# boomluo02/EEMFlow

Measured on AMD Instinct MI355X. Metric: frames/sec + EPE, EEMFlow 1280×720 dt1, 1/2/4/8 MI355X, higher is better.
Workload: dtype f32; 1 GPU; EEMFlow inference, HREM 1280x720 dt1, batch=1 per GPU (BASELINE configs[1]); synthetic 20%-dense voxel pairs resident in HBM, seeded Kaiming weights; height=720, width=1280, batch_per_gpu=1, hip_graph=True, streams_per_gpu=2, coalesced_frames=10, frames_in_flight_hint=2, preheat_steps=200, input_pairs_rotated=8, input_bytes_rotated=294912000, parallelism=replicas x1: frames sharded over ranks, no data-path collective

## Files before the change

eemflow_amd/_lib.py:

```python
import ctypes
import os

_HERE = os.path.dirname(os.path.abspath(__file__))
LIB_PATH = os.environ.get("EEM_LIB_PATH") or os.path.join(_HERE, "libeemflow_hip.so")

_c_float_p = ctypes.c_void_p


class KernelStat(ctypes.Structure):
    _fields_ = [("name", ctypes.c_char * 48), ("flops", ctypes.c_double), ("bytes", ctypes.c_double),
                ("ms", ctypes.c_float), ("blocks", ctypes.c_int), ("pipe", ctypes.c_int), ("reserved", ctypes.c_int)]


_SIGNATURES = {
    "eemflow_abi_version": (ctypes.c_int, []),
    "eemflow_last_error": (ctypes.c_char_p, []),
    "eemflow_create": (ctypes.c_int, [ctypes.c_int, ctypes.POINTER(ctypes.c_void_p)]),
    "eemflow_destroy": (None, [ctypes.c_void_p]),
    "eemflow_load_weights": (ctypes.c_int, [ctypes.c_void_p, _c_float_p, ctypes.c_size_t, ctypes.c_int, ctypes.c_int]),
    "eemflow_update_weights": (ctypes.c_int, [ctypes.c_void_p, _c_float_p, ctypes.c_size_t, ctypes.c_void_p]),
    "eemflow_forward_train": (ctypes.c_int, [ctypes.c_void_p, _c_float_p, _c_float_p, ctypes.c_int, ctypes.c_int, ctypes.c_int,
                                             _c_float_p, ctypes.c_int, ctypes.c_int, ctypes.POINTER(ctypes.c_int64), ctypes.c_void_p]),
    "eemflow_backward": (ctypes.c_int, [ctypes.c_void_p, ctypes.c_int64, _c_float_p, _c_float_p, _c_float_p, _c_float_p,
                                        ctypes.c_void_p]),
    "eemflow_backward_forms": (ctypes.c_int, [ctypes.c_void_p, ctypes.c_char_p, ctypes.c_size_t]),
    "eemflow_sequence_loss": (ctypes.c_int, [_c_float_p, _c_float_p, _c_float_p, ctypes.c_int, ctypes.c_int, ctypes.c_int, ctypes.c_float,
                                             _c_float_p, ctypes.c_void_p, ctypes.c_void_p]),
    "eemflow_set_image_size": (ctypes.c_int, [ctypes.c_void_p, ctypes.c_int, ctypes.c_int, ctypes.POINTER(ctypes.c_int * 4)]),
    "eemflow_use_graph": (ctypes.c_int, [ctypes.c_void_p, ctypes.c_int]),
    "eemflow_set_frames_in_flight": (ctypes.c_int, [ctypes.c_void_p, ctypes.c_int]),
    "eemflow_set_deferred_input_norm": (ctypes.c_int, [ctypes.c_void_p, ctypes.c_int]),
    "eemflow_graph_stats": (ctypes.c_int, [ctypes.c_void_p, ctypes.POINTER(ctypes.c_longlong * 3)]),
    "eemflow_forward": (ctypes.c_int, [ctypes.c_void_p, _c_float_p, _c_float_p, ctypes.c_int, ctypes.c_int, ctypes.c_int,
                                       _c_float_p, ctypes.c_int, ctypes.c_int, ctypes.c_void_p]),
    "eemflow_forward_many": (ctypes.c_int, [ctypes.c_void_p, ctypes.c_int, ctypes.POINTER(ctypes.c_void_p), ctypes.POINTER(ctypes.c_void_p),
                                            ctypes.POINTER(ctypes.c_void_p), ctypes.c_int, ctypes.c_int, ctypes.c_int, ctypes.c_int,
                                            ctypes.c_void_p]),
    "eemflow_forward_stream": (ctypes.c_int, [ctypes.c_void_p, ctypes.c_int, ctypes.POINTER(ctypes.c_void_p), ctypes.POINTER(ctypes.c_void_p),
                                              ctypes.c_int, ctypes.c_int, ctypes.c_int, ctypes.c_int, ctypes.c_int, ctypes.c_void_p]),
    "eemflow_forward_stream_bidir": (ctypes.c_int, [ctypes.c_void_p, ctypes.c_int, ctypes.POINTER(ctypes.c_void_p), ctypes.POINTER(ctypes.c_void_p),
                                                    ctypes.POINTER(ctypes.c_void_p), ctypes.c_int, ctypes.c_int, ctypes.c_int, ctypes.c_int,
                                                    ctypes.c_int, ctypes.c_void_p]),
    "eemflow_stream_reset": (ctypes.c_int, [ctypes.c_void_p]),
    "eemflow_stream_pending": (ctypes.c_int, [ctypes.c_void_p, ctypes.POINTER(ctypes.c_int)]),
    "eemflow_time_kernels": (ctypes.c_int, [ctypes.c_void_p, _c_float_p, _c_float_p, ctypes.c_int, ctypes.c_int, ctypes.c_int,
                                            _c_float_p, ctypes.c_int, ctypes.c_int, ctypes.c_int, ctypes.POINTER(KernelStat),
                                            ctypes.c_int, ctypes.POINTER(ctypes.c_int), ctypes.c_void_p]),
    "eemflow_get_stage": (ctypes.c_int, [ctypes.c_void_p, ctypes.c_char_p, _c_float_p, ctypes.c_size_t,
                                         ctypes.POINTER(ctypes.c_int * 4), ctypes.c_void_p]),
    "eemflow_decoder": (ctypes.c_int, [ctypes.c_void_p, ctypes.c_int, _c_float_p, ctypes.c_int, ctypes.c_int, ctypes.c_int,
                                       _c_float_p, ctypes.c_void_p]),
    "eemflow_local_corr53": (ctypes.c_int, [_c_float_p, _c_float_p, ctypes.c_int, ctypes.c_int, ctypes.c_int, ctypes.c_int,
                                            _c_float_p, ctypes.c_void_p]),
    "eemflow_upsample_bilinear": (ctypes.c_int, [_c_float_p, _c_float_p, ctypes.c_int, ctypes.c_int, ctypes.c_int,
                                                 ctypes.c_int, ctypes.c_int, ctypes.c_void_p]),
    "eraft_corr_lookup_bwd": (ctypes.c_int, [_c_float_p, _c_float_p, ctypes.c_int, ctypes.c_int, ctypes.c_int, _c_float_p,
                                             _c_float_p, _c_float_p, _c_float_p, ctypes.c_void_p]),
    "eraft_corr_pyramid_bwd": (ctypes.c_int, [_c_float_p, _c_float_p, _c_float_p, _c_float_p, _c_float_p, _c_float_p, ctypes.c_int,
                                              ctypes.c_int, ctypes.c_int, ctypes.c_int, _c_float_p, _c_float_p, ctypes.c_void_p]),
    "eraft_convex_upsample_bwd": (ctypes.c_int, [_c_float_p, _c_float_p, _c_float_p, ctypes.c_int, ctypes.c_int, ctypes.c_int,
                                                 _c_float_p, _c_float_p, ctypes.c_void_p]),
    "eemplus_warp_bwd": (ctypes.c_int, [_c_float_p, _c_float_p, _c_float_p, ctypes.c_int, ctypes.c_int, ctypes.c_int, ctypes.c_int,
                                        ctypes.c_int, _c_float_p, _c_float_p, ctypes.c_void_p]),
    "eemflow_flow_error": (ctypes.c_int, [_c_float_p, _c_float_p, ctypes.c_void_p, ctypes.c_int, ctypes.c_int, ctypes.c_int,
# ... 144 lines not shown
```

eemflow_amd/csrc/api.hip:

```cpp
#include <stdarg.h>
#include <stdlib.h>
#include <string.h>

#include <string>
#include <vector>

#include "ctx.h"
#include <mutex>

static thread_local char g_err[512] = "";
thread_local int eem_last_grid_blocks = 0, eem_last_grid_threads = 0, eem_last_pipe = 0;

void eem_set_error(const char* fmt, ...) {
    va_list ap;
    va_start(ap, fmt);
    vsnprintf(g_err, sizeof(g_err), fmt, ap);
    va_end(ap);
}

extern "C" const char* eemflow_last_error(void) { return g_err; }
extern "C" int eemflow_abi_version(void) { return 1; }

extern "C" int eemflow_create(int device, eemflow_ctx** out) {
    EEM_REQUIRE(out != nullptr, "eemflow_create: out is NULL");
    int ndev = 0;
    EEM_HIP_CHECK(hipGetDeviceCount(&ndev));
    EEM_REQUIRE(device >= 0 && device < ndev, "eemflow_create: device %d of %d", device, ndev);
    EEM_HIP_CHECK(hipSetDevice(device));
    hipDeviceProp_t prop;
    EEM_HIP_CHECK(hipGetDeviceProperties(&prop, device));
    EEM_REQUIRE(strncmp(prop.gcnArchName, "gfx950", 6) == 0,
                "this library is built for gfx950 (MI355X) only; device %d is %s", device, prop.gcnArchName);
    eemflow_ctx* c = new eemflow_ctx();
    c->device = device;
    hipError_t e = hipMalloc(&c->taps, sizeof(kTaps53));
    if (e == hipSuccess) e = hipMemcpy(c->taps, kTaps53, sizeof(kTaps53), hipMemcpyHostToDevice);
    if (e == hipSuccess) e = hipMalloc(&c->zero_page, 4096);
    if (e == hipSuccess) e = hipMemset(c->zero_page, 0, 4096);
    if (e == hipSuccess) e = hipMalloc(&c->io_table, 3 * EEM_MAX_COALESCE * sizeof(void*));
    if (e == hipSuccess) e = hipMemset(c->io_table, 0, 3 * EEM_MAX_COALESCE * sizeof(void*));
    if (e != hipSuccess) {
        eem_set_error("eemflow_create: %s", hipGetErrorString(e));
        delete c;
        return EEM_ERR_HIP;
    }
    *out = c;
    return EEM_OK;
}

extern "C" void eemflow_destroy(eemflow_ctx* c) {
    if (!c) return;
    (void)hipSetDevice(c->device);
    drop_graph(c);
    DevBuf* bufs[] = {&c->a1, &c->f11, &c->a2, &c->b2, &c->f12, &c->a3, &c->b3, &c->f13, &c->flowcat, &c->coarse, &c->carry,
                      &c->padded, &c->fuse_scratch, &c->g_a1, &c->g_f11, &c->g_a2, &c->g_b2, &c->g_f12, &c->g_a3, &c->g_b3, &c->g_f13,
                      &c->g_flowcat, &c->g_coarse, &c->g_flow, &c->ups_tmp, &c->grad_flat, &c->adam_m, &c->adam_v, &c->scalars};
    for (DevBuf* b : bufs) if (b->p) (void)hipFree(b->p);
    for (int k = 0; k < 3; ++k) {
        if (c->ppart[k].p) (void)hipFree(c->ppart[k].p);
        DevBuf* kb[] = {&c->pool[k], &c->cat[k], &c->ta[k], &c->tb[k], &c->tc[k], &c->td[k], &c->t64[k], &c->t32[k],
                        &c->g_pool[k], &c->g_cat[k], &c->g_ta[k], &c->g_tb[k], &c->g_tc[k], &c->g_td[k], &c->g_t64[k], &c->g_t32[k]};
        for (DevBuf* b : kb) if (b->p) (void)hipFree(b->p);
    }
    if (c->cstream) { (void)hipStreamSynchronize(c->cstream); (void)hipStreamDestroy(c->cstream); }
// ... 725 lines not shown
```

eemflow_amd/csrc/common.h:

```cpp
#pragma once
#include <hip/hip_runtime.h>
#include <cstdio>
#include <cstdlib>
#include <stdint.h>
#include <stdio.h>

#include <type_traits>

#include "../../include/eemflow_hip.h"

typedef float f32x2 __attribute__((ext_vector_type(2)));
typedef float f32x4 __attribute__((ext_vector_type(4)));
typedef float f32x16 __attribute__((ext_vector_type(16)));
typedef double f64x2 __attribute__((ext_vector_type(2)));
typedef unsigned u32x4 __attribute__((ext_vector_type(4)));

#define EEM_OK 0
#define EEM_ERR_ARG 1
#define EEM_ERR_HIP 2
#define EEM_ERR_STATE 3

void eem_set_error(const char* fmt, ...);

extern thread_local const char* eem_conv_form;

#define EEM_HIP_CHECK(expr)                                                            \
    do {                                                                               \
        hipError_t _e = (expr);                                                        \
        if (_e != hipSuccess) {                                                        \
            eem_set_error("%s failed: %s (%s:%d)", #expr, hipGetErrorString(_e),       \
                          __FILE__, __LINE__);                                         \
            return EEM_ERR_HIP;                                                        \
        }                                                                              \
    } while (0)

#define EEM_REQUIRE(cond, ...)                                                         \
    do {                                                                               \
        if (!(cond)) {                                                                 \
            eem_set_error(__VA_ARGS__);                                                \
            return EEM_ERR_ARG;                                                        \
        }                                                                              \
    } while (0)

__host__ __device__ static inline int ceil_div(int a, int b) { return (a + b - 1) / b; }

extern thread_local int eem_last_grid_blocks, eem_last_grid_threads, eem_last_pipe;
#define EEM_NOTE_GRID(blocks, threads) do { eem_last_grid_blocks = (int)(blocks); eem_last_grid_threads = (int)(threads); } while (0)
#define EEM_NOTE_PIPE(p) do { eem_last_pipe = (int)(p); } while (0)

template <int I, int N, class F>
__device__ __forceinline__ void static_for(F&& f) {
    if constexpr (I < N) {
        f(std::integral_constant<int, I>{});
        static_for<I + 1, N>(f);
    }
}
template <int N>
__device__ __forceinline__ void wait_vmcnt() {
    asm volatile("s_waitcnt vmcnt(%0)" ::"n"(N > 63 ? 63 : N) : "memory");
}

__device__ static inline unsigned xcd_logical_block(unsigned bid, unsigned nblocks_padded) {
    const unsigned cpx = nblocks_padded >> 3;
    return (bid & 7u) * cpx + (bid >> 3);
}

template <int CTRL>
__device__ static __forceinline__ float dpp_add(float v) {
    return v + __int_as_float(__builtin_amdgcn_update_dpp(0, __float_as_int(v), CTRL, 0xF, 0xF, true));
}
template <int SW>
__device__ static __forceinline__ float lane_group_sum(float v) {
    static_assert(SW == 4 || SW == 8 || SW == 16, "group width");
    v = dpp_add<0xB1>(v);
    v = dpp_add<0x4E>(v);
    if (SW >= 8) v = dpp_add<0x141>(v);
    if (SW >= 16) v = dpp_add<0x140>(v);
    return v;
}

static inline int enc_blocks_per_xcd(const char* tag, int dflt) {
    char name[48];
    snprintf(name, sizeof name, "EEM_ENC_PER_XCD_%s", tag);
    const char* e = getenv(name);
    if (!e) e = getenv("EEM_ENC_PER_XCD");
    const int v = e ? atoi(e) : 0;
    return v > 0 ? v : dflt;
}
struct TileCoord { int bx, by, n; };
struct TileRange { int first, count; };
__device__ static inline TileRange block_tile_range(int T, unsigned bid, unsigned nblocks) {
    const int cpx = (T + 7) >> 3;
    const int xcd = bid & 7, kb = bid >> 3, gb = nblocks >> 3;
    const int r0 = xcd * cpx, r1 = min(r0 + cpx, T);
    const int per = (cpx + gb - 1) / gb;
    const int f = r0 + kb * per;
    const int cnt = min(per, r1 - f);
    return TileRange{f, cnt > 0 ? cnt : 0};
}
__device__ static inline TileCoord tile_coord(int lt, int tiles_x, int tiles_y) {
    return TileCoord{lt % tiles_x, (lt / tiles_x) % tiles_y, lt / (tiles_x * tiles_y)};
// ... 217 lines not shown
```

eemflow_amd/csrc/conv_bx3.hip:

```cpp
#include "common.h"

namespace {

#define LDS_PTR(p) ((__attribute__((address_space(3))) void*)(p))
#define GLB_PTR(p) ((const __attribute__((address_space(1))) void*)(p))

typedef unsigned u32x4 __attribute__((ext_vector_type(4)));
typedef __bf16 bf16x8 __attribute__((ext_vector_type(8)));

template <int CIN, int COUT>
struct BxCfg {
    static constexpr int TH = 4, NPIX = 32, WAVES = 4;
    static constexpr int MT = COUT / 32;
    static constexpr int NC16 = CIN / 16;
    static constexpr int KSTEPS = 9 * NC16;
    static constexpr int IN_ROWS = 2 * (TH - 1) + 3;
    static constexpr int ROWP = 68;
    static constexpr int PPR = ROWP / 4;
    static constexpr int PLANE = IN_ROWS * ROWP;
    static constexpr int PIECES = CIN * IN_ROWS * PPR;
    static constexpr int NI = (PIECES + WAVES * 64 - 1) / (WAVES * 64);
    static constexpr int LDS_FLOATS = NI * WAVES * 256;
    static constexpr int RING = 3;
};

__device__ __forceinline__ bf16x8 as_bf(const u32x4& v) { return __builtin_bit_cast(bf16x8, v); }

__device__ __forceinline__ void split8(const float (&x)[8], u32x4& p0, u32x4& p1, u32x4& p2) {
#pragma unroll
    for (int d = 0; d < 4; ++d) {
        const float xa = x[2 * d], xb = x[2 * d + 1];
        const float ra = xa - __uint_as_float(__float_as_uint(xa) & 0xffff0000u), rb = xb - __uint_as_float(__float_as_uint(xb) & 0xffff0000u);
        const float sa = ra - __uint_as_float(__float_as_uint(ra) & 0xffff0000u), sb = rb - __uint_as_float(__float_as_uint(rb) & 0xffff0000u);
        p0[d] = __builtin_amdgcn_perm(__float_as_uint(xb), __float_as_uint(xa), 0x07060302u);
        p1[d] = __builtin_amdgcn_perm(__float_as_uint(rb), __float_as_uint(ra), 0x07060302u);
        p2[d] = __builtin_amdgcn_perm(__float_as_uint(sb), __float_as_uint(sa), 0x07060302u);
    }
}

__device__ __forceinline__ void split_pair(const float (&x)[8], int d, u32x4& p0, u32x4& p1, u32x4& p2) {
    const float xa = x[2 * d], xb = x[2 * d + 1];
    const float ra = xa - __uint_as_float(__float_as_uint(xa) & 0xffff0000u), rb = xb - __uint_as_float(__float_as_uint(xb) & 0xffff0000u);
    const float sa = ra - __uint_as_float(__float_as_uint(ra) & 0xffff0000u), sb = rb - __uint_as_float(__float_as_uint(rb) & 0xffff0000u);
    p0[d] = __builtin_amdgcn_perm(__float_as_uint(xb), __float_as_uint(xa), 0x07060302u);
    p1[d] = __builtin_amdgcn_perm(__float_as_uint(rb), __float_as_uint(ra), 0x07060302u);
    p2[d] = __builtin_amdgcn_perm(__float_as_uint(sb), __float_as_uint(sa), 0x07060302u);
}

template <int CIN, int COUT>
__global__ __launch_bounds__(256, (CIN == 16 ? 4 : 2)) void bx3_s2_kernel(EncConvArgs a, const u32x4* __restrict__ wq) {
    using C = BxCfg<CIN, COUT>;
    __shared__ __attribute__((aligned(16))) float lds[C::LDS_FLOATS];
    const int tid = threadIdx.x;
    const int lane = tid & 63;
    const int wave = __builtin_amdgcn_readfirstlane(tid >> 6);
    ENC_ARGS_NOW(a);
    const unsigned lid = xcd_logical_block(blockIdx.x, gridDim.x);
    if (lid >= (unsigned)(a.tiles_x * a.tiles_y * a.nimg)) return;
    const int bx = lid % a.tiles_x, by = (lid / a.tiles_x) % a.tiles_y;
    const int n = lid / (a.tiles_x * a.tiles_y);
    const int row = wave;
    const int j = lane & 31, g = lane >> 5;

    const u32x4* wsrc = wq + lane;
    u32x4 wv[C::RING][3][C::MT];
#pragma unroll
    for (int s = 0; s < C::RING; ++s)
#pragma unroll
        for (int p = 0; p < 3; ++p)
#pragma unroll
            for (int m = 0; m < C::MT; ++m) wv[s][p][m] = wsrc[((s * 3 + p) * C::MT + m) * 64];

    const int oy0 = by * C::TH, ox0 = bx * C::NPIX;
    const int gy0 = oy0 * 2 - 1, gxa = ox0 * 2 - 4;
    const float* src = a.in0 + (size_t)n * CIN * a.hin * a.win;
#pragma unroll
    for (int k = 0; k < C::NI; ++k) {
// ... 23 lines not shown
        for (int e = 0; e < 8; ++e) x[e] = bl[(c16 * 16 + e) * C::PLANE + (t / 3) * C::ROWP + (t % 3)];
    };
    asm volatile("s_waitcnt vmcnt(0)" ::: "memory");
    __builtin_amdgcn_s_barrier();
    float x[2][8];
    u32x4 b[2][3];
    read_x(0, x[0]);
    if (C::KSTEPS > 1) read_x(1, x[1]);
    split8(x[0], b[0][0], b[0][1], b[0][2]);
#pragma unroll
    for (int s = 0; s < C::KSTEPS; ++s) {
        const int cur = s & 1, nxt = cur ^ 1;
        u32x4(&w)[3][C::MT] = wv[s % C::RING];
        if (s + 2 < C::KSTEPS) read_x(s + 2, x[cur]);
        __builtin_amdgcn_sched_barrier(0);
#pragma unroll
        for (int q = 0; q < 6; ++q) {
            constexpr int PW[6] = {2, 1, 0, 1, 0, 0}, PB[6] = {0, 1, 2, 0, 1, 0};
#pragma unroll
            for (int m = 0; m < C::MT; ++m)
                acc[m] = __builtin_amdgcn_mfma_f32_32x32x16_bf16(as_bf(w[PW[q]][m]), as_bf(b[cur][PB[q]]), acc[m], 0, 0, 0);
            if (q < 4 && s + 1 < C::KSTEPS) split_pair(x[nxt], q, b[nxt][0], b[nxt][1], b[nxt][2]);
            __builtin_amdgcn_sched_barrier(0);
        }
        if (s + C::RING < C::KSTEPS) {
#pragma unroll
            for (int p = 0; p < 3; ++p)
#pragma unroll
                for (int m = 0; m < C::MT; ++m) w[p][m] = wsrc[(((s + C::RING) * 3 + p) * C::MT + m) * 64];
        }
        __builtin_amdgcn_sched_barrier(0);
    }

    const int oy = oy0 + row, ox = ox0 + j;
    const int hw = a.hout * a.wout;
    float* dst = a.out + (size_t)n * COUT * hw;
    const bool full = oy0 + C::TH <= a.hout && ox0 + C::NPIX <= a.wout;
#pragma unroll
    for (int m = 0; m < C::MT; ++m) {
        const int co0 = m * 32 + 4 * g;
        const unsigned lane_bo = (unsigned)((co0 * a.hout + oy) * a.wout + ox) * 4u;
#pragma unroll
        for (int r = 0; r < 16; ++r) {
            float v = acc[m][r];
            if (a.act) v = fmaxf(v, 0.1f * v);
            const int dco = (r & 3) + 8 * (r >> 2);
            if (full) {
                char* rb = reinterpret_cast<char*>(dst) + (size_t)dco * hw * 4;
                *reinterpret_cast<float*>(rb + lane_bo) = v;
            } else if (oy < a.hout && ox < a.wout) {
                dst[(size_t)(co0 + dco) * hw + oy * a.wout + ox] = v;
            }
        }
    }
}

__global__ void bx3_wt_kernel(const float* __restrict__ w, int cin, int cout, unsigned* __restrict__ out, int total) {
    const int i = blockIdx.x * blockDim.x + threadIdx.x;
    if (i >= total) return;
    const int nc16 = cin / 16, mt_n = cout / 32;
    const int d = i & 3, lane = (i >> 2) & 63;
    int rest = i >> 8;
    const int mt = rest % mt_n; rest /= mt_n;
    const int s = rest;
    const int t = s / nc16, c16 = s % nc16;
    const int co = mt * 32 + (lane & 31), c = c16 * 16 + 8 * (lane >> 5) + 2 * d;
    unsigned lo[3], hi[3];
    for (int h = 0; h < 2; ++h) {
        const float x = w[((size_t)co * cin + c + h) * 9 + t];
        const float x0 = __uint_as_float(__float_as_uint(x) & 0xffff0000u), r = x - x0;
        const float x1 = __uint_as_float(__float_as_uint(r) & 0xffff0000u), q = r - x1;
        unsigned* dst = h ? hi : lo;
        dst[0] = __float_as_uint(x0) >> 16; dst[1] = __float_as_uint(x1) >> 16; dst[2] = __float_as_uint(q) >> 16;
    }
    for (int p = 0; p < 3; ++p) out[((((size_t)s * 3 + p) * mt_n + mt) * 64 + lane) * 4 + d] = (hi[p] << 16) | lo[p];
}

template <int CIN, int COUT, int KGT>
struct B1Cfg {
    static constexpr int TH = 4, NPIX = 32, KG = KGT, WAVES = 4 * KG, THREADS = 64 * WAVES;
    static constexpr int MT = COUT / 32;
    static constexpr int NC16 = CIN / 16, NCG = NC16 / KG;
    static constexpr int KLOC = 9 * NCG;
    static constexpr int NG = CIN / 8;
    static constexpr int IN_ROWS = TH + 2, COLS = 40, QPR = COLS / 4;
    static constexpr int ITEMS = NG * IN_ROWS * QPR;
    static constexpr int GPLANE = IN_ROWS * COLS;
    static constexpr int TILE_U4 = 3 * NG * GPLANE;
    static constexpr int SLOT_U4 = 3 * MT * 64;
    static constexpr int NQ = 3 * MT;
    static constexpr int RING = KG == 1 ? 6 : 4, AHEAD = RING - 1;
    static constexpr int LDS_U4 = TILE_U4 + KG * RING * SLOT_U4;
    static_assert(ITEMS <= THREADS && NC16 % KG == 0 && NQ <= 8 && (KG == 1 || MT == 2), "one staging item per thread; two groups finish one cout tile each");
    static_assert(KG == 1 || MT * 4 * 64 * 4 <= TILE_U4, "partial-sum exchange fits the dead input tile");
    static_assert(LDS_U4 * 16 <= 160 * 1024, "LDS");
};

template <int N>
__device__ __forceinline__ void bx_wait_vm(int nrow) {
    if (nrow == 2) asm volatile("s_waitcnt vmcnt(%0)" ::"n"(2 * N) : "memory");
    else if (nrow == 1) asm volatile("s_waitcnt vmcnt(%0)" ::"n"(N) : "memory");
    else asm volatile("s_waitcnt vmcnt(0)" ::: "memory");
}

template <int CIN, int COUT, int KGT>
__global__ __launch_bounds__((64 * 4 * KGT), (KGT == 1 ? 2 : 1)) void bx3_s1_kernel(EncConvArgs a, const u32x4* __restrict__ wq) {
// ... 104 lines not shown
        f32x16* xch = reinterpret_cast<f32x16*>(lds);
        xch[((1 - kg) * 4 + row) * 64 + lane] = kg == 0 ? acc[1] : acc[0];
        __syncthreads();
        f32x16 mine = kg == 0 ? acc[0] : acc[1];
        const f32x16 other = xch[(kg * 4 + row) * 64 + lane];
        const int co0 = kg * 32 + 4 * g;
        if (oy < a.hout && ox < a.wout) {
#pragma unroll
            for (int r = 0; r < 16; ++r) {
                const int co = co0 + (r & 3) + 8 * (r >> 2);
                float v = mine[r] + other[r] + a.bias[co];
                if (a.act) v = fmaxf(v, 0.1f * v);
                dst[(size_t)co * hw + oy * a.wout + ox] = v;
            }
        }
    } else {
        if (oy < a.hout && ox < a.wout) {
#pragma unroll
            for (int m = 0; m < C::MT; ++m)
#pragma unroll
                for (int r = 0; r < 16; ++r) {
                    const int co = m * 32 + 4 * g + (r & 3) + 8 * (r >> 2);
                    float v = acc[m][r] + a.bias[co];
                    if (a.act) v = fmaxf(v, 0.1f * v);
                    dst[(size_t)co * hw + oy * a.wout + ox] = v;
                }
        }
    }
}

template <int CIN, int COUT, int KGT>
int bx3_s1_launch_t(const EncConvArgs& a0, hipStream_t stream) {
    using C = B1Cfg<CIN, COUT, KGT>;
    EncConvArgs a = a0;
    a.tiles_x = ceil_div(a.wout, C::NPIX);
    a.tiles_y = ceil_div(a.hout, C::TH);
    dim3 grid((unsigned)ceil_div(a.tiles_x * a.tiles_y * a.nimg, 8) * 8);
    EEM_NOTE_GRID(grid.x, C::THREADS);
    EEM_NOTE_PIPE(1);
    hipLaunchKernelGGL((bx3_s1_kernel<CIN, COUT, KGT>), grid, dim3(C::THREADS), 0, stream, a, reinterpret_cast<const u32x4*>(a.wbx3));
    EEM_HIP_CHECK(hipGetLastError());
    return EEM_OK;
}

template <int CIN, int COUT>
int bx3_launch_t(const EncConvArgs& a0, hipStream_t stream) {
    using C = BxCfg<CIN, COUT>;
    EncConvArgs a = a0;
    a.tiles_x = ceil_div(a.wout, C::NPIX);
    a.tiles_y = ceil_div(a.hout, C::TH);
    dim3 grid((unsigned)ceil_div(a.tiles_x * a.tiles_y * a.nimg, 8) * 8);
    EEM_NOTE_GRID(grid.x, 256);
    EEM_NOTE_PIPE(1);
    hipLaunchKernelGGL((bx3_s2_kernel<CIN, COUT>), grid, dim3(256), 0, stream, a, reinterpret_cast<const u32x4*>(a.wbx3));
    EEM_HIP_CHECK(hipGetLastError());
    return EEM_OK;
}

}

bool bx3_shape(int cin, int cout, int stride) {
    return (stride == 2 && ((cin == 16 && cout == 32) || (cin == 32 && cout == 64))) || (stride == 1 && cin == cout && (cin == 32 || cin == 64));
}

size_t bx3_packed_floats(int cin, int cout) { return (size_t)9 * (cin / 16) * 3 * (cout / 32) * 64 * 4; }

int bx3_transform_launch(const float* w, int cin, int cout, float* packed, hipStream_t stream) {
    const int total = 9 * (cin / 16) * (cout / 32) * 64 * 4;
    hipLaunchKernelGGL(bx3_wt_kernel, dim3(ceil_div(total, 256)), dim3(256), 0, stream, w, cin, cout, reinterpret_cast<unsigned*>(packed), total);
    EEM_HIP_CHECK(hipGetLastError());
    return EEM_OK;
}

bool bx3_supported(int cin, int cout, int stride, const EncConvArgs& a) {
    const char* off = getenv("EEM_NO_BX3");
    if (off && off[0] == '1') return false;
    if (stride == 2 && cin == 32) {
        const char* m = getenv("EEM_NO_BX3_64");
        if (m && m[0] == '1') return false;
    }
    if (stride == 1) {
        const char* m = getenv("EEM_BX3_S1");
        const int mask = m ? atoi(m) : 0;
        if (!(mask & (cin == 32 ? 1 : 2))) return false;
    }
    return bx3_shape(cin, cout, stride) && a.wbx3 && a.gate == nullptr && a.pool_partial == nullptr && a.res == nullptr && (a.win & 3) == 0 &&
           (a.act == 0 || a.act == 1) && (((uintptr_t)a.in0) & 15) == 0 && (size_t)cin * a.hin * a.win * 4 < (1u << 31);
}

int bx3_launch(int cin, int stride, const EncConvArgs& a, hipStream_t stream) {
    if (cin == 64) return bx3_s1_launch_t<64, 64, 2>(a, stream);
    if (cin == 32 && stride == 2) return bx3_launch_t<32, 64>(a, stream);
    if (cin == 32) return bx3_s1_launch_t<32, 32, 1>(a, stream);
    return bx3_launch_t<16, 32>(a, stream);
}
```

eemflow_amd/csrc/ctx.h:

```cpp
#pragma once
#include <stdarg.h>
#include <string.h>

#include <string>
#include <vector>

#include "../../include/eemflow_hip.h"
#include "common.h"
#include "gconv.h"
#include "eraft_kernels.h"
#include "wnc.h"

inline constexpr int kTaps53[53] = {0,  2,  4,  6,  8,  10, 12, 14, 16, 18, 20, 21, 22, 23, 24, 26, 28, 29,
                                    30, 31, 32, 33, 34, 36, 38, 39, 40, 41, 42, 44, 46, 47, 48, 49, 50, 51,
                                    52, 54, 56, 57, 58, 59, 60, 62, 64, 66, 68, 70, 72, 74, 76, 78, 80};
constexpr int kNTaps = 53;
constexpr int kDecIn = kNTaps + 16;
constexpr int kDecW = 100;

struct TailW {
    size_t wpk = 0, bias = 0;
    int cin = 0, cout = 0, ksize = 3;
};

// ... 119 lines not shown
        int stream_nvol = 0;
        int stream_carry = 0, stream_slot = 0;
        int stream_bidir = 0;
        bool operator==(const Key& o) const {
            return batch == o.batch && in_h == o.in_h && in_w == o.in_w && out_h == o.out_h && out_w == o.out_w &&
                   pad[0] == o.pad[0] && pad[1] == o.pad[1] && pad[2] == o.pad[2] && pad[3] == o.pad[3] && aligned16 == o.aligned16 &&
                   io_frames == o.io_frames && deferred_norm == o.deferred_norm && stream_nvol == o.stream_nvol &&
                   stream_carry == o.stream_carry && stream_slot == o.stream_slot && stream_bidir == o.stream_bidir;
        }
    };
    struct GraphEntry {
        Key key;
        Shape shape;
        bool f13_skipped = false;
        bool a1_skipped = false;
        hipGraph_t graph = nullptr;
        hipGraphExec_t exec = nullptr;
        long last_use = 0;
    };
    static constexpr int kMaxGraphs = 4;
    std::vector<GraphEntry> graphs;
    long graph_clock = 0;
    const void** io_table = nullptr;
    const void* io_host[3 * EEM_MAX_COALESCE] = {};
    int io_host_n = 0;
    int cur_io_frames = 0;
    void* io_stream = nullptr;
    long graph_captures = 0, graph_replays = 0, io_updates = 0;
};

struct Hook {
    hipStream_t st = nullptr;
    bool timing = false;
    int reps = 1;
    bool repeat = false;
    int pass = 0;
    size_t slot = 0;
    std::vector<hipEvent_t> evs;
    std::vector<eemflow_kernel_stat> stats;

    static bool skipped(const char* name);

    template <class F>
    int run(const char* name, double flops, double bytes, F&& launch) {
#ifdef EEM_DIAG
        if (skipped(name)) {
            static const float spin = [] { const char* e = getenv("EEM_SKIP_SPIN_US"); return e ? (float)atof(e) : 0.f; }();
            return spin > 0.f ? spin_launch(spin, st) : EEM_OK;
        }
#endif
        if (!timing) return launch(st);
        if (repeat) {
            if (evs.size() < 2) { evs.resize(2, nullptr); EEM_HIP_CHECK(hipEventCreate(&evs[0])); EEM_HIP_CHECK(hipEventCreate(&evs[1])); }
            eem_last_grid_blocks = eem_last_grid_threads = eem_last_pipe = 0;
            int rc = launch(st);
            if (rc != EEM_OK) return rc;
            EEM_HIP_CHECK(hipEventRecord(evs[0], st));
            for (int i = 0; i < reps; ++i)
                if ((rc = launch(st)) != EEM_OK) return rc;
            EEM_HIP_CHECK(hipEventRecord(evs[1], st));
            EEM_HIP_CHECK(hipEventSynchronize(evs[1]));
            float ms = 0.f;
            EEM_HIP_CHECK(hipEventElapsedTime(&ms, evs[0], evs[1]));
            eemflow_kernel_stat ks;
            memset(&ks, 0, sizeof(ks));
            strncpy(ks.name, name, sizeof(ks.name) - 1);
            ks.flops = flops; ks.bytes = bytes; ks.ms = ms;
            ks.blocks = eem_last_grid_blocks;
            ks.pipe = eem_last_pipe;
            stats.push_back(ks);
            return EEM_OK;
        }
        if (evs.size() < 2 * (slot + 1)) {
            evs.resize(2 * (slot + 1), nullptr);
            EEM_HIP_CHECK(hipEventCreate(&evs[2 * slot]));
            EEM_HIP_CHECK(hipEventCreate(&evs[2 * slot + 1]));
        }
        eem_last_grid_blocks = eem_last_grid_threads = eem_last_pipe = 0;
        EEM_HIP_CHECK(hipEventRecord(evs[2 * slot], st));
        const int rc = launch(st);
        if (rc != EEM_OK) return rc;
        EEM_HIP_CHECK(hipEventRecord(evs[2 * slot + 1], st));
        if (pass == 0) {
            eemflow_kernel_stat ks;
            memset(&ks, 0, sizeof(ks));
            strncpy(ks.name, name, sizeof(ks.name) - 1);
            ks.flops = flops; ks.bytes = bytes; ks.ms = 0.f;
            ks.blocks = eem_last_grid_blocks;
            ks.pipe = eem_last_pipe;
            stats.push_back(ks);
        }
        ++slot;
        return EEM_OK;
    }
    int collect(bool count);
    void release();
};

extern thread_local unsigned long g_realloc_events;
int ensure(DevBuf& b, size_t floats);
int refresh_wino(eemflow_ctx* c, hipStream_t);
int ensure_bx3(eemflow_ctx* c, int l, hipStream_t st, const float** w_out);
int ensure_s2r(eemflow_ctx* c, int l, hipStream_t st, const float** w_out);
int ensure_wino(eemflow_ctx* c, int l, int dir, int batch, hipStream_t st, const float** w_out, int* f4_out);
int ensure_dec_wnc(eemflow_ctx* c, hipStream_t st);
int ensure_train_wino(eemflow_ctx* c, int batch, hipStream_t st);
int ensure_forward_wino(eemflow_ctx* c, int batch, hipStream_t st);
void drop_graph(eemflow_ctx* c);
int compute_shape(eemflow_ctx* c, int batch, int in_h, int in_w, int out_h, int out_w, Shape* s, int nimg = -1);
int alloc_workspace(eemflow_ctx* c, const Shape& s);

bool s2r_wanted();
bool bx3_wanted(int l);
bool dec_wnc_wanted(const eemflow_ctx* c, int gw, int batch);
int run_decoders(eemflow_ctx* c, int k0, int k1, const float* const cat[3], int batch, int h, int w, float* flow_dst,
                 int flow_ctotal, int kbase, Hook& hk);
int run_enc_layer(eemflow_ctx* c, const Shape& s, int li, const float* e1, const float* e2, Hook& hk, const void* const* io,
                  const float* prepadded, bool may_skip_store);
int run_forward(eemflow_ctx* c, const Shape& s, const float* e1, const float* e2, float* out, Hook& hk,
                const void* const* io = nullptr, const float* prepadded = nullptr);
```

include/eemflow_hip.h:

```cpp
#ifndef EEMFLOW_HIP_H
#define EEMFLOW_HIP_H

#include <stddef.h>
#include <stdint.h>

#ifdef __cplusplus
extern "C" {
#endif
typedef struct eemflow_ctx eemflow_ctx;
typedef struct eraft_ctx eraft_ctx;
typedef struct eemplus_ctx eemplus_ctx;

#if defined(__GNUC__)
#pragma GCC visibility push(default)
#endif

int eemflow_abi_version(void);

const char* eemflow_last_error(void);

int eemflow_create(int device, eemflow_ctx** out);
void eemflow_destroy(eemflow_ctx* ctx);

int eemflow_load_weights(eemflow_ctx* ctx, const float* flat_host, size_t nfloats, int n_first_channels,
                         int groups);

int eemflow_update_weights(eemflow_ctx* ctx, const float* flat_device, size_t nfloats, void* stream);

int eemflow_set_image_size(eemflow_ctx* ctx, int height, int width, int pad_out[4]);

int eemflow_use_graph(eemflow_ctx* ctx, int enable);

int eemflow_set_frames_in_flight(eemflow_ctx* ctx, int n);

int eemflow_set_deferred_input_norm(eemflow_ctx* ctx, int enable);

int eemflow_graph_stats(eemflow_ctx* ctx, long long out3[3]);

int eemflow_forward(eemflow_ctx* ctx, const float* events1, const float* events2, int batch, int in_h,
                    int in_w, float* flow_out, int out_h, int out_w, void* stream);

int eemflow_forward_many(eemflow_ctx* ctx, int nframes, const float* const* events1, const float* const* events2,
                         float* const* flow_out, int in_h, int in_w, int out_h, int out_w, void* stream);

#define EEM_STREAM_MAX_VOLUMES 16

int eemflow_forward_stream(eemflow_ctx* ctx, int nvol, const float* const* volumes, float* const* flow_out, int nflow, int in_h,
                           int in_w, int out_h, int out_w, void* stream);

#define EEM_STREAM_BIDIR_MAX_VOLUMES 8

int eemflow_forward_stream_bidir(eemflow_ctx* ctx, int nvol, const float* const* volumes, float* const* flow_fw_out,
                                 float* const* flow_bw_out, int nflow, int in_h, int in_w, int out_h, int out_w, void* stream);

int eemflow_stream_reset(eemflow_ctx* ctx);

int eemflow_stream_pending(eemflow_ctx* ctx, int* out);

typedef struct eemflow_kernel_stat {
    char name[48];
    double flops;
    double bytes;
    float ms;
    int blocks;
    int pipe;
    int reserved;
} eemflow_kernel_stat;
int eemflow_time_kernels(eemflow_ctx* ctx, const float* events1, const float* events2, int batch, int in_h,
                         int in_w, float* flow_out, int out_h, int out_w, int reps, eemflow_kernel_stat* stats,
                         int max_stats, int* nstats, void* stream);

int eemflow_get_stage(eemflow_ctx* ctx, const char* name, float* dst, size_t dst_capacity_floats,
                      int dims_out[4], void* stream);

int eemflow_decoder(eemflow_ctx* ctx, int k, const float* x, int batch, int h, int w, float* out, void* stream);

int eemflow_local_corr53(const float* f1, const float* f2, int batch, int c, int h, int w, float* out,
                         void* stream);

int eemflow_upsample_bilinear(const float* in, float* out, int nc, int h, int w, int oh, int ow, void* stream);

int eemflow_flow_error(const float* flow_gt, const float* flow_pred, const float* event_img, int h, int w, int max_row,
                       double* out5, void* stream);

int eemflow_flow_error_many(int n, const float* const* flow_gt, const float* const* flow_pred, const float* const* event_img, int h,
                            int w, int max_row, double* out5n, void* stream);

int eemflow_fb_check_many(int n, const float* const* flow_fw, const float* const* flow_bw, float* const* mask_fw_out,
                          float* const* mask_bw_out, int h, int w, float alpha1, float alpha2, int mode, void* stream);

int eemflow_flow_to_image_many(int n, const float* const* flow, uint8_t* const* image_out, double* stats, int h, int w, int bgr,
                               void* stream);

int eemflow_event_image_many(int n, const float* const* volume, const float* const* norm, int bins, int h, int w,
                             uint8_t* const* image_out, double* stats, int bgr, void* stream);

int eemflow_voxelize(const double* events, int64_t n, int bins, int h, int w, int normalize, float* grid,
                     int64_t* idx_left, int64_t* idx_right, void* stream);

int eemflow_voxelize_pair(const double* events1, int64_t n1, const double* events2, int64_t n2, int bins, int h, int w,
                          int normalize, float* grid1, float* grid2, void* stream);

int eemflow_voxelize_many(int nsets, const double* const* events, const int64_t* n_events, int bins, int h, int w, int normalize,
                          float* const* grids, void* stream);


int eemflow_forward_train(eemflow_ctx* ctx, const float* events1, const float* events2, int batch, int in_h, int in_w,
                          float* flow_out, int out_h, int out_w, int64_t* serial_out, void* stream);
int eemflow_backward(eemflow_ctx* ctx, int64_t serial, const float* events1, const float* events2, const float* dflow,
                     float* grad_out, void* stream);

int eemflow_backward_forms(eemflow_ctx* ctx, char* dst, size_t capacity);

int eemflow_sequence_loss(const float* flow, const float* flow_gt, const float* valid, int batch, int h, int w, float weight,
                          float* dflow_out, double* stats6, void* stream);

int eemflow_forward_backward(eemflow_ctx* ctx, const float* events1, const float* events2, const float* flow_gt,
                             const float* valid, int batch, int in_h, int in_w, int out_h, int out_w,
                             float loss_weight, float* flow_out, float* grad_out, double* stats_out, void* stream);
// ... 154 lines not shown
```

Measured before the change: 11050 frames/s.

## Add lean stride-2 bx3 conv kernel with padded LDS planes and packed split

```diff
diff --git a/eemflow_amd/_lib.py b/eemflow_amd/_lib.py
--- a/eemflow_amd/_lib.py
+++ b/eemflow_amd/_lib.py
@@ -9,7 +9,7 @@
 
 class KernelStat(ctypes.Structure):
     _fields_ = [("name", ctypes.c_char * 48), ("flops", ctypes.c_double), ("bytes", ctypes.c_double),
-                ("ms", ctypes.c_float), ("blocks", ctypes.c_int), ("pipe", ctypes.c_int), ("reserved", ctypes.c_int)]
+                ("ms", ctypes.c_float), ("blocks", ctypes.c_int), ("pipe", ctypes.c_int), ("form", ctypes.c_int)]
 
 
 _SIGNATURES = {
diff --git a/eemflow_amd/csrc/api.hip b/eemflow_amd/csrc/api.hip
--- a/eemflow_amd/csrc/api.hip
+++ b/eemflow_amd/csrc/api.hip
@@ -9,7 +9,7 @@
 #include <mutex>
 
 static thread_local char g_err[512] = "";
-thread_local int eem_last_grid_blocks = 0, eem_last_grid_threads = 0, eem_last_pipe = 0;
+thread_local int eem_last_grid_blocks = 0, eem_last_grid_threads = 0, eem_last_pipe = 0, eem_last_form = 0;
 
 void eem_set_error(const char* fmt, ...) {
     va_list ap;
diff --git a/eemflow_amd/csrc/common.h b/eemflow_amd/csrc/common.h
--- a/eemflow_amd/csrc/common.h
+++ b/eemflow_amd/csrc/common.h
@@ -44,9 +44,10 @@
 
 __host__ __device__ static inline int ceil_div(int a, int b) { return (a + b - 1) / b; }
 
-extern thread_local int eem_last_grid_blocks, eem_last_grid_threads, eem_last_pipe;
+extern thread_local int eem_last_grid_blocks, eem_last_grid_threads, eem_last_pipe, eem_last_form;
 #define EEM_NOTE_GRID(blocks, threads) do { eem_last_grid_blocks = (int)(blocks); eem_last_grid_threads = (int)(threads); } while (0)
 #define EEM_NOTE_PIPE(p) do { eem_last_pipe = (int)(p); } while (0)
+#define EEM_NOTE_FORM(f) do { eem_last_form = (int)(f); } while (0)
 
 template <int I, int N, class F>
 __device__ __forceinline__ void static_for(F&& f) {
diff --git a/eemflow_amd/csrc/conv_bx3.hip b/eemflow_amd/csrc/conv_bx3.hip
--- a/eemflow_amd/csrc/conv_bx3.hip
+++ b/eemflow_amd/csrc/conv_bx3.hip
@@ -22,7 +22,31 @@
     static constexpr int NI = (PIECES + WAVES * 64 - 1) / (WAVES * 64);
     static constexpr int LDS_FLOATS = NI * WAVES * 256;
     static constexpr int RING = 3;
+    static constexpr int PLANE_L = 640;
+    static constexpr int PPL = PLANE_L / 4;
+    static constexpr int PERIOD = 5;
+    static_assert(CIN * PPL == NI * WAVES * 64 && CIN * PLANE_L == LDS_FLOATS, "the padded planes fill today's LDS exactly");
+    static_assert(PERIOD * WAVES * 64 == 8 * PPL && NI % PERIOD == 0, "five rounds are eight planes");
+    static_assert((CIN - 9) * (PLANE_L / 64) <= 255, "read2st64 offsets (channel c16 * 16 + e; 8 g is the lane's) are 8 bits of 64-dword strides");
 };
+
+struct BxPiece { unsigned c, ry, q; };
+__host__ __device__ constexpr BxPiece bx_piece(unsigned p) {
+    const unsigned c = (((p >> 5) & 0xffu) * 205u) >> 10;
+    unsigned rem = p - c * 160u;
+    rem = rem < 152u ? rem : 152u;
+    const unsigned ry = (rem * 241u) >> 12;
+    return BxPiece{c, ry, rem - ry * 17u};
+}
+constexpr bool bx_piece_check() {
+    for (unsigned p = 0; p < 32 * 160; ++p) {
+        const BxPiece x = bx_piece(p);
+        const unsigned rem = p % 160 < 152 ? p % 160 : 152;
+        if (x.c != p / 160 || x.ry != rem / 17 || x.q != rem % 17) return false;
+    }
+    return true;
+}
+static_assert(bx_piece_check(), "bx_piece");
 
 __device__ __forceinline__ bf16x8 as_bf(const u32x4& v) { return __builtin_bit_cast(bf16x8, v); }
 
@@ -152,6 +176,155 @@
                 dst[(size_t)(co0 + dco) * hw + oy * a.wout + ox] = v;
             }
         }
+    }
+}
+
+__device__ __forceinline__ void split_pk(const f32x2 x, int d, u32x4& p0, u32x4& p1, u32x4& p2) {
+    typedef unsigned u32x2 __attribute__((ext_vector_type(2)));
+    const f32x2 r = x - __builtin_bit_cast(f32x2, __builtin_bit_cast(u32x2, x) & 0xffff0000u);
+    const f32x2 q = r - __builtin_bit_cast(f32x2, __builtin_bit_cast(u32x2, r) & 0xffff0000u);
+    p0[d] = __builtin_amdgcn_perm(__float_as_uint(x[1]), __float_as_uint(x[0]), 0x07060302u);
+    p1[d] = __builtin_amdgcn_perm(__float_as_uint(r[1]), __float_as_uint(r[0]), 0x07060302u);
+    p2[d] = __builtin_amdgcn_perm(__float_as_uint(q[1]), __float_as_uint(q[0]), 0x07060302u);
+}
+
+template <int CIN, int COUT>
+__global__ __launch_bounds__(256, (CIN == 16 ? 4 : 2)) void bx3_s2_lean_kernel(EncConvArgs a, const u32x4* __restrict__ wq) {
+    using C = BxCfg<CIN, COUT>;
+    __shared__ __attribute__((aligned(16))) float lds[C::LDS_FLOATS];
+    const int tid = threadIdx.x;
+    const int lane = tid & 63;
+    const int wave = __builtin_amdgcn_readfirstlane(tid >> 6);
+    ENC_ARGS_NOW(a);
+    const unsigned lid = xcd_logical_block(blockIdx.x, gridDim.x);
+    if (lid >= (unsigned)(a.tiles_x * a.tiles_y * a.nimg)) return;
+    const int bx = lid % a.tiles_x, by = (lid / a.tiles_x) % a.tiles_y;
+    const int n = lid / (a.tiles_x * a.tiles_y);
+    const int row = wave;
+    const int j = lane & 31, g = lane >> 5;
+
+    const u32x4* wsrc = wq + lane;
+    u32x4 wv[C::RING][3][C::MT];
+#pragma unroll
+    for (int s = 0; s < C::RING; ++s)
+#pragma unroll
+        for (int p = 0; p < 3; ++p)
+#pragma unroll
+            for (int m = 0; m < C::MT; ++m) wv[s][p][m] = wsrc[((s * 3 + p) * C::MT + m) * 64];
+
+    const int oy0 = by * C::TH, ox0 = bx * C::NPIX;
+    const int gy0 = oy0 * 2 - 1, gxa = ox0 * 2 - 4;
+    const unsigned row_b = (unsigned)a.win * 4u, plane_b = (unsigned)a.hin * row_b;
+    const char* org = reinterpret_cast<const char*>(a.in0) + (size_t)n * CIN * plane_b + ((long)gy0 * a.win + gxa) * 4;
+    const size_t step_b = (size_t)8 * plane_b;
+    unsigned off[C::PERIOD];
+    BxPiece pc[C::PERIOD];
+#pragma unroll
+    for (int k = 0; k < C::PERIOD; ++k) {
+        pc[k] = bx_piece((unsigned)((wave + k * C::WAVES) * 64 + lane));
+        off[k] = pc[k].c * plane_b + __umul24(pc[k].ry, row_b) + pc[k].q * 16u;
+    }
+    const bool interior = gy0 >= 0 && gy0 + C::IN_ROWS <= a.hin && gxa >= 0 && gxa + C::ROWP <= a.win;
+    if (interior) {
+#pragma unroll
+        for (int k = 0; k < C::NI; ++k)
+            __builtin_amdgcn_global_load_lds(GLB_PTR(org + (k / C::PERIOD) * step_b + off[k % C::PERIOD]), LDS_PTR(lds + (wave + k * C::WAVES) * 256), 16, 0, 0);
+    } else {
+        const unsigned rymin = gy0 < 0 ? -gy0 : 0, nry = (unsigned)min(C::IN_ROWS, a.hin - gy0) - rymin;
+        const unsigned qmin = gxa < 0 ? (-gxa) >> 2 : 0, nq = (unsigned)min(C::PPR, (a.win - gxa) >> 2) - qmin;
+        const char* zero_page = reinterpret_cast<const char*>(a.zero_page);
+        bool ok[C::PERIOD];
+#pragma unroll
+        for (int k = 0; k < C::PERIOD; ++k) ok[k] = pc[k].ry - rymin < nry && pc[k].q - qmin < nq;
+#pragma unroll
+        for (int k = 0; k < C::NI; ++k) {
+            const char* gp = org + (k / C::PERIOD) * step_b + off[k % C::PERIOD];
+            gp = ok[k % C::PERIOD] ? gp : zero_page;
+            __builtin_amdgcn_global_load_lds(GLB_PTR(gp), LDS_PTR(lds + (wave + k * C::WAVES) * 256), 16, 0, 0);
+        }
+    }
+
+    f32x16 acc[C::MT];
+#pragma unroll
+    for (int m = 0; m < C::MT; ++m)
+#pragma unroll
+        for (int r = 0; r < 16; ++r) acc[m][r] = a.bias[m * 32 + (r & 3) + 8 * (r >> 2) + 4 * g];
+
+    int boff = (g * 8 * C::PLANE_L + 2 * row * C::ROWP + 2 * j + 3) * 4;
+    int btap = 0;
+    auto read_x = [&](int s, f32x2 (&x)[4]) __attribute__((always_inline)) {
+        const int t = s / C::NC16, c16 = s % C::NC16;
+        if (t != btap) {
+            boff += (((t / 3) * C::ROWP + t % 3) - ((btap / 3) * C::ROWP + btap % 3)) * 4;
+            asm volatile("" : "+v"(boff));
+            btap = t;
+        }
+        const float* bt = reinterpret_cast<const float*>(reinterpret_cast<const char*>(lds) + boff);
+#pragma unroll
+        for (int d = 0; d < 4; ++d) x[d] = f32x2{bt[(c16 * 16 + 2 * d) * C::PLANE_L], bt[(c16 * 16 + 2 * d + 1) * C::PLANE_L]};
+    };
+    asm volatile("s_waitcnt vmcnt(0)" ::: "memory");
+    __builtin_amdgcn_s_barrier();
+    f32x2 x[2][4];
+    u32x4 b[2][3];
+    read_x(0, x[0]);
+    if (C::KSTEPS > 1) read_x(1, x[1]);
+#pragma unroll
+    for (int d = 0; d < 4; ++d) split_pk(x[0][d], d, b[0][0], b[0][1], b[0][2]);
+#pragma unroll
+    for (int s = 0; s < C::KSTEPS; ++s) {
+        const int cur = s & 1, nxt = cur ^ 1;
+        u32x4(&w)[3][C::MT] = wv[s % C::RING];
+        if (s + 2 < C::KSTEPS) read_x(s + 2, x[cur]);
+        __builtin_amdgcn_sched_barrier(0);
+#pragma unroll
+        for (int q = 0; q < 6; ++q) {
+            constexpr int PW[6] = {2, 1, 0, 1, 0, 0}, PB[6] = {0, 1, 2, 0, 1, 0};
+#pragma unroll
+            for (int m = 0; m < C::MT; ++m)
+                acc[m] = __builtin_amdgcn_mfma_f32_32x32x16_bf16(as_bf(w[PW[q]][m]), as_bf(b[cur][PB[q]]), acc[m], 0, 0, 0);
+            if (q < 4 && s + 1 < C::KSTEPS) split_pk(x[nxt][q], q, b[nxt][0], b[nxt][1], b[nxt][2]);
+            __builtin_amdgcn_sched_barrier(0);
+        }
+        if (s + C::RING < C::KSTEPS) {
+#pragma unroll
+            for (int p = 0; p < 3; ++p)
+#pragma unroll
+                for (int m = 0; m < C::MT; ++m) w[p][m] = wsrc[(((s + C::RING) * 3 + p) * C::MT + m) * 64];
+        }
+        __builtin_amdgcn_sched_barrier(0);
+    }
+
+    const int oy = oy0 + row, ox = ox0 + j;
+    const int hw = a.hout * a.wout;
+    float* dst = a.out + (size_t)n * COUT * hw;
+    if (oy0 + C::TH <= a.hout && ox0 + C::NPIX <= a.wout) {
+        const unsigned lane_bo = (unsigned)((4 * g * a.hout + oy) * a.wout + ox) * 4u;
+        const size_t hw4 = (size_t)hw * 4;
+        auto store_all = [&](auto act) __attribute__((always_inline)) {
+            char* rb = reinterpret_cast<char*>(dst);
+#pragma unroll
+            for (int m = 0; m < C::MT; ++m)
+#pragma unroll
+                for (int r = 0; r < 16; ++r) {
+                    float v = acc[m][r];
+                    if (decltype(act)::value) v = fmaxf(v, 0.1f * v);
+                    *reinterpret_cast<float*>(rb + lane_bo) = v;
+                    rb += (r & 3) == 3 ? 5 * hw4 : hw4;
+                }
+        };
+        if (a.act) store_all(std::true_type{});
+        else store_all(std::false_type{});
+    } else if (oy < a.hout && ox < a.wout) {
+        float* lp = dst + (size_t)(4 * g) * hw + oy * a.wout + ox;
+#pragma unroll
+        for (int m = 0; m < C::MT; ++m)
+#pragma unroll
+            for (int r = 0; r < 16; ++r) {
+                float v = acc[m][r];
+                if (a.act) v = fmaxf(v, 0.1f * v);
+                lp[(size_t)(m * 32 + (r & 3) + 8 * (r >> 2)) * hw] = v;
+            }
     }
 }
 
@@ -362,7 +535,11 @@
     dim3 grid((unsigned)ceil_div(a.tiles_x * a.tiles_y * a.nimg, 8) * 8);
     EEM_NOTE_GRID(grid.x, 256);
     EEM_NOTE_PIPE(1);
-    hipLaunchKernelGGL((bx3_s2_kernel<CIN, COUT>), grid, dim3(256), 0, stream, a, reinterpret_cast<const u32x4*>(a.wbx3));
+    const char* form = getenv("EEM_BX3_S2_FORM");
+    const bool lean = !(form && form[0] == '0') && a.win < (1 << 22);
+    EEM_NOTE_FORM(lean ? 1 : 0);
+    if (lean) hipLaunchKernelGGL((bx3_s2_lean_kernel<CIN, COUT>), grid, dim3(256), 0, stream, a, reinterpret_cast<const u32x4*>(a.wbx3));
+    else hipLaunchKernelGGL((bx3_s2_kernel<CIN, COUT>), grid, dim3(256), 0, stream, a, reinterpret_cast<const u32x4*>(a.wbx3));
     EEM_HIP_CHECK(hipGetLastError());
     return EEM_OK;
 }
diff --git a/eemflow_amd/csrc/ctx.h b/eemflow_amd/csrc/ctx.h
--- a/eemflow_amd/csrc/ctx.h
+++ b/eemflow_amd/csrc/ctx.h
@@ -195,7 +195,7 @@
         if (!timing) return launch(st);
         if (repeat) {
             if (evs.size() < 2) { evs.resize(2, nullptr); EEM_HIP_CHECK(hipEventCreate(&evs[0])); EEM_HIP_CHECK(hipEventCreate(&evs[1])); }
-            eem_last_grid_blocks = eem_last_grid_threads = eem_last_pipe = 0;
+            eem_last_grid_blocks = eem_last_grid_threads = eem_last_pipe = eem_last_form = 0;
             int rc = launch(st);
             if (rc != EEM_OK) return rc;
             EEM_HIP_CHECK(hipEventRecord(evs[0], st));
@@ -211,6 +211,7 @@
             ks.flops = flops; ks.bytes = bytes; ks.ms = ms;
             ks.blocks = eem_last_grid_blocks;
             ks.pipe = eem_last_pipe;
+            ks.form = eem_last_form;
             stats.push_back(ks);
             return EEM_OK;
         }
@@ -219,7 +220,7 @@
             EEM_HIP_CHECK(hipEventCreate(&evs[2 * slot]));
             EEM_HIP_CHECK(hipEventCreate(&evs[2 * slot + 1]));
         }
-        eem_last_grid_blocks = eem_last_grid_threads = eem_last_pipe = 0;
+        eem_last_grid_blocks = eem_last_grid_threads = eem_last_pipe = eem_last_form = 0;
         EEM_HIP_CHECK(hipEventRecord(evs[2 * slot], st));
         const int rc = launch(st);
         if (rc != EEM_OK) return rc;
@@ -231,6 +232,7 @@
             ks.flops = flops; ks.bytes = bytes; ks.ms = 0.f;
             ks.blocks = eem_last_grid_blocks;
             ks.pipe = eem_last_pipe;
+            ks.form = eem_last_form;
             stats.push_back(ks);
         }
         ++slot;
diff --git a/include/eemflow_hip.h b/include/eemflow_hip.h
--- a/include/eemflow_hip.h
+++ b/include/eemflow_hip.h
@@ -64,7 +64,7 @@
     float ms;
     int blocks;
     int pipe;
-    int reserved;
+    int form;
 } eemflow_kernel_stat;
 int eemflow_time_kernels(eemflow_ctx* ctx, const float* events1, const float* events2, int batch, int in_h,
                          int in_w, float* flow_out, int out_h, int out_w, int reps, eemflow_kernel_stat* stats,
```

New measurement: 11130 frames/s, median of 6. No clear change (+0.7%).
